# nvlong21/Lightweight-face-detection-CenterNet

Measured on AMD Instinct MI355X. Metric: images/sec at 640x640 batch inference, higher is better.
Workload: dtype bf16; 1 GPU; BASELINE configs[1]: batch=64 640x640 bf16 on 1 MI355X per rank, forward + top-100 peak decode; synthetic uint8 images resident in HBM, calibrated synthetic weights (seed 0); 2 context(s) per GPU, batch k on context k mod 2; batch_per_gpu=64, global_batch=64, topk=100, parallelism=dp1, contexts_per_gpu=2, input_buffers=4

## Files before the change

lightweight-face-detection-centernet_amd/csrc/cf_common.h:

```cpp
#pragma once
#include <hip/hip_runtime.h>
#include <stdint.h>
#include <stdlib.h>

typedef uint16_t bf16_t;

typedef __attribute__((ext_vector_type(4))) float f32x4;
typedef __attribute__((ext_vector_type(16))) float f32x16;
typedef __attribute__((ext_vector_type(8))) short bf16x8_t;
typedef __attribute__((ext_vector_type(4))) uint32_t u32x4;
typedef __attribute__((ext_vector_type(2))) uint32_t u32x2;

#define CF_WAVE 64

__device__ __forceinline__ float bf16_to_f32(uint32_t bits16) { return __uint_as_float(bits16 << 16); }
__device__ __forceinline__ float bf16lo(uint32_t packed) { return __uint_as_float(packed << 16); }
__device__ __forceinline__ float bf16hi(uint32_t packed) { return __uint_as_float(packed & 0xffff0000u); }

__device__ __forceinline__ uint32_t pack_bf16x2(float lo, float hi) {
    uint32_t r;
    asm("v_cvt_pk_bf16_f32 %0, %1, %2" : "=v"(r) : "v"(lo), "v"(hi));
    return r;
}

__device__ __forceinline__ float fast_rcp(float x) { return __builtin_amdgcn_rcpf(x); }

__device__ __forceinline__ float swish_f(float x) {
    return x * fast_rcp(1.0f + __expf(-x));
}
__device__ __forceinline__ float relu_f(float x) { return fmaxf(x, 0.0f); }

typedef __attribute__((ext_vector_type(2))) float f32x2;
__device__ __forceinline__ f32x2 swish2(f32x2 x) {
    const f32x2 t = x * -1.44269504088896341f;
    f32x2 e; e.x = __builtin_amdgcn_exp2f(t.x); e.y = __builtin_amdgcn_exp2f(t.y);
    const f32x2 den = e + 1.0f;
    f32x2 r; r.x = __builtin_amdgcn_rcpf(den.x); r.y = __builtin_amdgcn_rcpf(den.y);
    return x * r;
}
static constexpr float kCfNegLog2e = -1.44269504088896341f, kCfNegLn2 = -0.69314718055994531f;
template <bool PRE> __device__ __forceinline__ f32x2 swish2_sel(f32x2 x) {
    if constexpr (PRE) {
        f32x2 e; e.x = __builtin_amdgcn_exp2f(x.x); e.y = __builtin_amdgcn_exp2f(x.y);
        const f32x2 den = e + 1.0f;
        f32x2 r; r.x = __builtin_amdgcn_rcpf(den.x); r.y = __builtin_amdgcn_rcpf(den.y);
        return x * r;
    } else {
        return swish2(x);
    }
}
__device__ __forceinline__ f32x2 fma2(f32x2 a, f32x2 b, f32x2 c) { return __builtin_elementwise_fma(a, b, c); }
template <int ACT, int N> __device__ __forceinline__ void act_arr(float* v) {
    if constexpr (ACT == 1) {
#pragma unroll
        for (int e = 0; e < N; e += 2) {
            f32x2 x2; x2.x = v[e]; x2.y = v[e + 1];
            const f32x2 y2 = swish2(x2);
            v[e] = y2.x; v[e + 1] = y2.y;
        }
    } else if constexpr (ACT == 2) {
#pragma unroll
        for (int e = 0; e < N; ++e) v[e] = relu_f(v[e]);
    }
}
template <int ACT> __device__ __forceinline__ float act_f(float x) {
    if constexpr (ACT == 1) return swish_f(x);
    else if constexpr (ACT == 2) return relu_f(x);
    else return x;
}

template <typename T> struct Elem;
template <> struct Elem<float> {
    static constexpr int PER16 = 4;
};
template <> struct Elem<bf16_t> {
    static constexpr int PER16 = 8;
};

struct sp32_t { float v; };
template <> struct Elem<sp32_t> {
    static constexpr int PER16 = 4;
};

template <typename T> __device__ __forceinline__ void unpack16(const u32x4& c, float* f);
template <> __device__ __forceinline__ void unpack16<float>(const u32x4& c, float* f) {
    f[0] = __uint_as_float(c.x); f[1] = __uint_as_float(c.y);
// ... 92 lines not shown
typedef __attribute__((ext_vector_type(8))) uint32_t u32x8_t;
__device__ __forceinline__ void dot8_first(float* A, const u32x8_t& W, const u32x4& E0, const u32x4& E1) {
    asm("v_dot2_f32_f16 %0, %8, %16, 0\n\t"
        "v_dot2_f32_f16 %1, %9, %17, 0\n\t"
        "v_dot2_f32_f16 %2, %10, %18, 0\n\t"
        "v_dot2_f32_f16 %3, %11, %19, 0\n\t"
        "v_dot2_f32_f16 %4, %12, %20, 0\n\t"
        "v_dot2_f32_f16 %5, %13, %21, 0\n\t"
        "v_dot2_f32_f16 %6, %14, %22, 0\n\t"
        "v_dot2_f32_f16 %7, %15, %23, 0\n\t"
        "s_nop 2"
        : "=&v"(A[0]), "=&v"(A[1]), "=&v"(A[2]), "=&v"(A[3]), "=&v"(A[4]), "=&v"(A[5]), "=&v"(A[6]), "=&v"(A[7])
        : "s"(W[0]), "s"(W[1]), "s"(W[2]), "s"(W[3]), "s"(W[4]), "s"(W[5]), "s"(W[6]), "s"(W[7]),
          "v"(E0.x), "v"(E0.y), "v"(E0.z), "v"(E0.w), "v"(E1.x), "v"(E1.y), "v"(E1.z), "v"(E1.w));
}

__device__ __forceinline__ void cf_sync_lds_dma() {
    asm volatile("s_waitcnt vmcnt(0)" ::: "memory");
    __syncthreads();
}

template <int N> __device__ __forceinline__ void cf_sync_lds_dma_keep() {
    static_assert(N >= 0 && N <= 63, "vmcnt field");
    asm volatile("s_waitcnt vmcnt(%0)" :: "n"(N) : "memory");
    __syncthreads();
}

template <int DIV, int N, int SH = 16>
struct MulShiftDiv {
    static constexpr unsigned MUL = ((1u << SH) + DIV - 1) / DIV;
    static constexpr bool exact() {
        for (unsigned v = 0; v < (unsigned)N; ++v) if (((v * MUL) >> SH) != v / DIV) return false;
        return true;
    }
    static_assert((unsigned long long)N * MUL < (1ull << 32) && N < (1 << 24) && MUL < (1u << 24) && exact(), "24-bit multiply, exact quotient");
    static __device__ __forceinline__ unsigned div(unsigned v) { return (v * MUL) >> SH; }
};

typedef __amdgpu_buffer_rsrc_t cf_rsrc_t;
typedef __attribute__((ext_vector_type(4))) unsigned int cf_v4u;
constexpr unsigned CF_OOB = 0x80000000u;
__device__ __forceinline__ cf_rsrc_t cf_rsrc(const void* base, unsigned bytes) {
    return __builtin_amdgcn_make_buffer_rsrc(const_cast<void*>(base), 0, (int)bytes, 0x00020000);
}
__device__ __forceinline__ u32x4 cf_bload16(cf_rsrc_t r, unsigned off) {
    return __builtin_bit_cast(u32x4, __builtin_amdgcn_raw_buffer_load_b128(r, (int)off, 0, 0));
}
__device__ __forceinline__ uint32_t cf_bload4(cf_rsrc_t r, unsigned off) {
    return (uint32_t)__builtin_amdgcn_raw_buffer_load_b32(r, (int)off, 0, 0);
}
__device__ __forceinline__ void cf_bstore16(const u32x4& v, cf_rsrc_t r, unsigned off) {
    __builtin_amdgcn_raw_buffer_store_b128(__builtin_bit_cast(cf_v4u, v), r, (int)off, 0, 0);
}

template <int KS>
struct HaloDeal {
    static_assert(KS == 3 || KS == 5, "an even halo height");
    static constexpr int IH = 16 + KS - 1, IWQ = 5, NRP = IH / 2, NBLK = KS == 3 ? 3 : 4;
    static __device__ __forceinline__ int side_pairs(int w) { return w == 2 ? 4 : NRP - 4; }
    static __device__ __forceinline__ bool pixel(int w, int t, int pl, int& ty, int& tx) {
        const int tq = pl >> 3, hh = (pl >> 2) & 1, x = pl & 3;
        bool live = true;
        if (t < 2) {
            ty = 2 * (4 * t + w) + hh; tx = 4 * tq + x;
        } else if constexpr (KS == 3) {
            const bool side = w >= 2;
            const int lp = 2 * tq + (x >> 1);
            live = side ? lp < side_pairs(w) : tq < 2;
            ty = (side ? 2 * (4 * (w - 2) + lp) : 16) + hh;
            tx = side ? 16 + (x & 1) : 8 * w + 4 * tq + x;
        } else if (t == 2) {
            const bool side = w >= 2;
            ty = 2 * (side ? 4 * (w - 2) + tq : 8 + w) + hh;
            tx = side ? 16 + x : 4 * tq + x;
        } else {
            live = w >= 2 && tq == 0;
            ty = 2 * (6 + w) + hh; tx = 16 + x;
        }
        ty = live ? ty : 0; tx = live ? tx : 0;
        return live;
    }
};

template <int S, int TOH, int TOW, int IWP>
struct LaneMap {
    static constexpr int NPIX = TOH * TOW, PPX = S == 1 ? NPIX / 2 : NPIX, WPP = (PPX + 63) / 64, NSLOT = WPP * 64;
    static constexpr int ROWW = S == 1 ? TOW / 2 : TOW;
    static_assert(ROWW <= 64 && TOH <= 256, "entry packing: 6 bits of x, 9 bits of y below the idle flag");
    uint16_t v[NSLOT];
    static constexpr int pair_index(int r) {
        const int oy = r / ROWW, oxh = r - oy * ROWW;
        return S == 1 ? oy * (IWP / 2) + oxh : oy * IWP + oxh;
    }
    constexpr LaneMap() : v() {
        constexpr int NG = NSLOT / 16;
        int bucket[16][PPX] = {}; int cnt[16] = {}, used[16] = {};
        for (int r = 0; r < PPX; ++r) { const int b = pair_index(r) & 15; bucket[b][cnt[b]++] = r; }
        int slot[NSLOT] = {};
        for (int g = 0; g < NG; ++g)
            for (int b = 0; b < 16; ++b) slot[g * 16 + b] = used[b] < cnt[b] ? bucket[b][used[b]++] : -1;
        for (int b = 0; b < 16; ++b)
            while (used[b] < cnt[b]) {
                int s = 0; while (slot[s] >= 0) ++s;
                slot[s] = bucket[b][used[b]++];
            }
        for (int g = 0; g < NG; ++g)
            for (int j = 0; j < 16; ++j) {
                const int hw = g & 3;
                const int base = (hw & 1) ? (j < 8 ? 4 + j : j < 12 ? 16 + (j - 8) : 28 + (j - 12))
                                          : (j < 4 ? j : j < 8 ? 12 + (j - 4) : 20 + (j - 8));
                const int lane = base + (hw >> 1) * 32;
                const int r = slot[g * 16 + j];
                const int rc = r >= 0 ? r : cnt[j] > 0 ? bucket[j][0] : 0;
                const int oy = rc / ROWW, oxh = rc - oy * ROWW;
                v[(g >> 2) * 64 + lane] = (uint16_t)((r < 0 ? 0x8000 : 0) | (oy << 6) | oxh);
            }
    }
};

__device__ __forceinline__ int lds_group_pixel(int pl) {
    return pl < 4 ? pl : pl < 12 ? pl + 12 : pl < 16 ? pl - 8 : pl < 20 ? pl + 8 : pl < 28 ? pl - 12 : pl;
}

__device__ __forceinline__ void xcd_tile_order(unsigned& bx, unsigned& by, unsigned& bz) {
    const unsigned gx = gridDim.x, gy = gridDim.y, n = gx * gy * gridDim.z;
    unsigned l = blockIdx.x + gx * (blockIdx.y + gy * blockIdx.z);
    if ((n & 7u) == 0u) l = (l & 7u) * (n >> 3) + (l >> 3);
    bx = l % gx; l /= gx; by = l % gy; bz = l / gy;
}

static inline int cf_env_int(const char* name, int dflt) { const char* v = getenv(name); return v ? atoi(v) : dflt; }
#ifdef CF_EXPERIMENTS
static inline int cf_ab_int(const char* name, int dflt) { return cf_env_int(name, dflt); }
#else
static inline int cf_ab_int(const char*, int dflt) { return dflt; }
#endif

template <auto KFN, typename... A>
static inline hipError_t launch_lds(dim3 grid, dim3 blk, size_t lds, hipStream_t s, const A&... args) {
    if (lds > 64 * 1024) {
        static thread_local size_t raised_dev[32] = {};
        int dev = 0; (void)hipGetDevice(&dev);
        size_t& raised = raised_dev[dev & 31];
        if (raised < lds) {
            hipError_t e = hipFuncSetAttribute(reinterpret_cast<const void*>(KFN), hipFuncAttributeMaxDynamicSharedMemorySize, (int)lds);
            if (e != hipSuccess) return e;
            raised = lds;
        }
    }
    hipLaunchKernelGGL(KFN, grid, blk, lds, s, args...);
    return hipGetLastError();
}

template <typename E, size_t N, typename Match>
static inline const E* pick_variant(const E (&table)[N], int want, Match&& match) {
    const E* base = nullptr;
    for (const E& e : table)
        if (match(e)) {
            if (e.var == want) return &e;
            if (e.var == 0) base = &e;
        }
    return base;
}

static inline uint16_t host_f32_to_bf16(float f) {
    uint32_t u; __builtin_memcpy(&u, &f, 4);
// ... 41 lines not shown
```

lightweight-face-detection-centernet_amd/csrc/cf_mbconv2.hip:

```cpp
#include "cf_exp.h"
#include "cf_common.h"
#include "cf_kernels.h"
#include <cstdlib>
#include <type_traits>

namespace cf {

typedef __attribute__((ext_vector_type(8))) __bf16 mfma_bf16x8;
typedef __attribute__((ext_vector_type(8))) uint32_t u32x8;
typedef __attribute__((ext_vector_type(2))) __fp16 f16x2;
#define CF_AS4 __attribute__((address_space(4)))

static inline int slot_channel2(int nb, int i) {
    int h = (i >> 2) & 1;
    int r = (i & 3) + 4 * (i >> 3);
    return nb * 32 + h * 16 + r;
}

static inline uint16_t host_f32_to_f16(float f) {
    uint32_t u; __builtin_memcpy(&u, &f, 4);
    const uint32_t sign = (u >> 16) & 0x8000u;
    const int32_t exp = (int32_t)((u >> 23) & 0xff) - 127 + 15;
    uint32_t man = u & 0x7fffffu;
    if (((u >> 23) & 0xff) == 0xff) return (uint16_t)(sign | 0x7c00u | (man ? 0x200u : 0));
    if (exp >= 31) return (uint16_t)(sign | 0x7bffu);
    if (exp <= 0) {
        if (exp < -10) return (uint16_t)sign;
        man |= 0x800000u;
        const int shift = 14 - exp;
        uint32_t half = man >> shift;
        const uint32_t rem = man & ((1u << shift) - 1), mid = 1u << (shift - 1);
        if (rem > mid || (rem == mid && (half & 1))) ++half;
        return (uint16_t)(sign | half);
    }
    uint32_t half = ((uint32_t)exp << 10) | (man >> 13);
    const uint32_t rem = man & 0x1fffu;
    if (rem > 0x1000u || (rem == 0x1000u && (half & 1))) ++half;
    if (half >= 0x7c00u) half = 0x7bffu;
    return (uint16_t)(sign | half);
}

typedef __attribute__((ext_vector_type(2))) _Float16 hf2;
__device__ __forceinline__ void dot2c(float& acc, uint32_t w, uint32_t e) {
    acc = __builtin_amdgcn_fdot2(__builtin_bit_cast(hf2, w), __builtin_bit_cast(hf2, e), acc, false);
}

__device__ __forceinline__ f32x2 swish2_prescaled(f32x2 u) {
    f32x2 e; e.x = __builtin_amdgcn_exp2f(u.x); e.y = __builtin_amdgcn_exp2f(u.y);
    const f32x2 den = e + 1.0f;
    f32x2 r; r.x = __builtin_amdgcn_rcpf(den.x); r.y = __builtin_amdgcn_rcpf(den.y);
    return u * r;
}
static constexpr float kNegLog2e = -1.44269504088896341f, kNegLn2 = -0.69314718055994531f;

#define CF_DOT8_ACC(A, W, E0, E1)                                                                        \
    dot2c(A[0], W[0], E0.x); dot2c(A[1], W[1], E0.y); dot2c(A[2], W[2], E0.z); dot2c(A[3], W[3], E0.w);  \
    dot2c(A[4], W[4], E1.x); dot2c(A[5], W[5], E1.y); dot2c(A[6], W[6], E1.z); dot2c(A[7], W[7], E1.w)
#define CF_DOT8_Z(A, W, E0, E1)                                                                          \
    do { _Pragma("unroll") for (int i_ = 0; i_ < 8; ++i_) A[i_] = 0.0f; CF_DOT8_ACC(A, W, E0, E1); } while (0)
#define CF_DOT8(FIRST, A, W, E0, E1)                                                                     \
    do { if constexpr (FIRST) dot8_first(A, W, E0, E1); else { CF_DOT8_ACC(A, W, E0, E1); } } while (0)

#ifndef CF_WDIRECT_COND
#define CF_WDIRECT_COND (KS == 5 && S == 2 && NW == 3)
#endif
template <int KS, int S, int HC, int TOH, int TOW, int JX, int NW>
struct Px {
    static constexpr int IH = (TOH - 1) * S + KS, IW0 = (TOW - 1) * S + KS, IWP = (IW0 + 1) & ~1;
    static constexpr int IPX = IH * IWP, NIB = (IPX + 31) / 32, NPAIR = IPX / 2;
    static constexpr int NT = (KS + 1) / 2, NPARW = S == 1 ? 2 : 1;
    static constexpr int NPIX = TOH * TOW, PPX = S == 1 ? NPIX / 2 : NPIX, WPP = (PPX + 63) / 64;
    static constexpr int NPP = NPARW * WPP, KG = NW / NPP;
    static constexpr int NBE = (HC + 31) / 32, HALF = HC / 16, JS = HALF / KG;
    static constexpr bool PART = (HC % 32 == 16);
    static constexpr int NBF = HC / 32;
    static constexpr int PITCH = HC * 4 + 16;
    static constexpr int WXB = (NBF * JX + (PART ? 1 : 0)) * 1024;
    static_assert(!PART || JX <= 2, "half block needs Cin <= 32");
    static constexpr int EBYTES = NIB * 16 * PITCH;
    static constexpr int RED = (KG - 1) * NPP * 64 * 64;
    static constexpr bool WDIRECT = CF_WDIRECT_COND;
    static constexpr int WLDS = WDIRECT ? 0 : 2 * WXB;
    static constexpr int LDS = (EBYTES + WLDS) > RED ? (EBYTES + WLDS) : RED;
    static_assert(NPP * KG == NW && TOW % 2 == 0, "tile / wave geometry");
    static_assert(HC % 16 == 0 && JS * KG == HALF, "hidden chunk / k-group geometry");
};

#ifndef CF_XRELOAD_COND
#define CF_XRELOAD_COND (KS == 5 && S == 2 && NBO == 1 && NW == 3)
#endif
template <int KS, int S, int NBO, bool RESID, int NW, int JX, int HC, int TOH, int TOW, int MODE = 0>
__global__ __launch_bounds__(NW * 64) void mbconv_px_kernel(MbParams p) {
    typedef Px<KS, S, HC, TOH, TOW, JX, NW> G;
    constexpr bool FAST = MODE != 0, FAST_LD = (MODE & 1) != 0, FAST_WR = (MODE & 2) != 0;
    static_assert(!FAST || (!RESID && !G::PART), "MODE != 0: no residual, no 16-channel half block");
    constexpr int IWP = G::IWP, IPX = G::IPX, NIB = G::NIB, NPAIR = G::NPAIR, NT = G::NT, NPARW = G::NPARW;
    constexpr int NPP = G::NPP, KG = G::KG, NBF = G::NBF, HALF = G::HALF, JS = G::JS, PITCH = G::PITCH, WXB = G::WXB;
    constexpr bool PART = G::PART;
    extern __shared__ __attribute__((aligned(16))) char smem[];
    char* E = smem;
    char* Wst = smem + G::EBYTES;

    const int tid = threadIdx.x, lane = tid & 63;
    const int wave = __builtin_amdgcn_readfirstlane(tid >> 6);
    const int pl = lane & 31, h = lane >> 5;
    unsigned tbx = blockIdx.x, tby = blockIdx.y, tbz = blockIdx.z;
    if (p.nw) xcd_tile_order(tbx, tby, tbz);
    const int ox0 = tbx * TOW, oy0 = tby * TOH, b = tbz;
    const int nq = p.nq;
    const int pp = wave % NPP, jg = wave / NPP;

    const int par = S == 1 ? pp / G::WPP : 0;
    static constexpr LaneMap<S, TOH, TOW, IWP> kLanes{};
    const int lm0 = (S == 1 ? pp - par * G::WPP : pp) * 64;
    auto tile_pixel = [&](int blk, int lane31, int& oy, int& ox) -> bool {
        const uint32_t e = kLanes.v[lm0 + blk * 32 + lane31];
        oy = (e >> 6) & 0x1ff;
        ox = S == 1 ? 2 * (int)(e & 63) + par : (int)(e & 63);
        return (e & 0x8000u) == 0;
    };
    int dy, dx; tile_pixel(h, pl, dy, dx);
    const unsigned e_pix = (unsigned)(((dy * S) * IWP + (dx * S - par)) / 2) * (unsigned)PITCH;

    f32x16 acc[2][NBO];
#pragma unroll
    for (int k = 0; k < 2; ++k)
#pragma unroll
        for (int i = 0; i < NBO; ++i)
#pragma unroll
            for (int r = 0; r < 16; ++r) acc[k][i][r] = 0.0f;

    const char* xbase = (const char*)p.x + (size_t)b * p.Hin * p.Win * p.Cin * 2;
    const unsigned rowbytes = (unsigned)p.Cin * 2;

    auto stage_weights = [&](int q) {
        char* dst = Wst + (q & 1) * WXB;
        const char* srcx = (const char*)p.wexp + (size_t)q * WXB;
        for (int c = wave; c < WXB / 1024; c += NW)
            __builtin_amdgcn_global_load_lds((const __attribute__((address_space(1))) void*)(srcx + c * 1024 + lane * 16),
                                             (__attribute__((address_space(3))) void*)(dst + c * 1024), 16, 0, 0);
    };

    constexpr int MAXI = (NIB + NW - 1) / NW;
    constexpr bool XRELOAD = CF_XRELOAD_COND;
    u32x4 xf[MAXI][JX];
    u32x4 xh[PART ? MAXI : 1][2];
    typedef MulShiftDiv<IWP, MAXI * NW * 32> HD;
    const unsigned ip0 = (unsigned)(wave * 32 + pl);
    const int gy0 = oy0 * S - p.pad_lo, gx0 = ox0 * S - p.pad_lo;
    const unsigned hlim = (unsigned)min(p.Hin, gy0 + G::IH);
    const unsigned lbase = (((unsigned)b * (unsigned)p.Hin + (unsigned)gy0) * (unsigned)p.Win + (unsigned)gx0) * rowbytes + (unsigned)(h * JX * 16);
    const unsigned pitch24 = ((unsigned)p.Win * rowbytes) & 0xffffffu, rowb24 = rowbytes & 0xffffffu;
    const unsigned oobh = (h && (p.Cin & 8)) ? CF_OOB : 0u;
    const cf_rsrc_t xr = cf_rsrc(p.x, FAST_LD ? (unsigned)p.B * (unsigned)p.Hin * (unsigned)p.Win * rowbytes : 0u);
    auto load_x = [&]() {
    if constexpr (FAST_LD) {
#pragma unroll
        for (int t = 0; t < MAXI; ++t) {
            const unsigned ip = ip0 + (unsigned)(t * NW * 32);
            const unsigned iy = HD::div(ip), ix = ip - iy * (unsigned)IWP;
            const bool valid = (unsigned)(gy0 + (int)iy) < hlim && (unsigned)(gx0 + (int)ix) < (unsigned)p.Win;
            const unsigned off = valid ? iy * pitch24 + (ix * rowb24 + lbase) : CF_OOB;
#pragma unroll
            for (int j = 0; j < JX; ++j) xf[t][j] = cf_bload16(xr, (j == JX - 1 ? (off | oobh) : off) + j * 16);
        }
        return;
    }
#pragma unroll
    for (int t = 0; t < MAXI; ++t) {
        const int ib = wave + NW * t;
        const int ip = ib * 32 + pl;
        const int ipc = ip < IPX ? ip : IPX - 1;
        const int iy = ipc / IWP, ix = ipc - iy * IWP;
        const int gy = oy0 * S - p.pad_lo + iy, gx = ox0 * S - p.pad_lo + ix;
        const bool valid = ip < IPX && (unsigned)gy < (unsigned)p.Hin && (unsigned)gx < (unsigned)p.Win;
        const int cy = min(max(gy, 0), p.Hin - 1), cx = min(max(gx, 0), p.Win - 1);
        const unsigned off = ((unsigned)cy * (unsigned)p.Win + (unsigned)cx) * rowbytes + (unsigned)(h * JX * 16);
#pragma unroll
        for (int j = 0; j < JX; ++j) {
            const bool vj = valid && (h * JX + j) * 8 < p.Cin;
            const u32x4 v = ld16(xbase + off + j * 16);
            xf[t][j].x = vj ? v.x : 0u; xf[t][j].y = vj ? v.y : 0u;
            xf[t][j].z = vj ? v.z : 0u; xf[t][j].w = vj ? v.w : 0u;
        }
    }

    if constexpr (PART) {
#pragma unroll
        for (int t = 0; t < MAXI; ++t)
#pragma unroll
            for (int sub = 0; sub < 2; ++sub) {
                const int ib = wave + NW * t;
                const int ip = ib * 32 + sub * 16 + (lane & 15), kg = lane >> 4;
                const int ipc = ip < IPX ? ip : IPX - 1;
                const int iy = ipc / IWP, ix = ipc - iy * IWP;
                const int gy = oy0 * S - p.pad_lo + iy, gx = ox0 * S - p.pad_lo + ix;
                const bool valid = ip < IPX && (unsigned)gy < (unsigned)p.Hin && (unsigned)gx < (unsigned)p.Win && kg * 8 < p.Cin;
                const int cy = min(max(gy, 0), p.Hin - 1), cx = min(max(gx, 0), p.Win - 1);
                const u32x4 v = ld16(xbase + ((unsigned)cy * (unsigned)p.Win + (unsigned)cx) * rowbytes + (unsigned)(min(kg * 8, p.Cin - 8) * 2));
                xh[t][sub].x = valid ? v.x : 0u; xh[t][sub].y = valid ? v.y : 0u;
                xh[t][sub].z = valid ? v.z : 0u; xh[t][sub].w = valid ? v.w : 0u;
            }
    }
    };
    if constexpr (!XRELOAD) load_x();

    constexpr int VP = (IPX - 32 * (NIB - 1)) / 2;
    auto expand_block = [&](auto lastb, int ib, const u32x4* xfr, const u32x4* xhr, const char* wx) {
        constexpr bool LASTB = decltype(lastb)::value && VP < 16;
        if constexpr (PART) {
            const u32x4 wv = ld16(wx + (NBF * JX * 64 + lane) * 16);
            char* ecol = E + (NBF * 32 + (lane & 15)) * 4 + (unsigned)(ib * 16 + 2 * (lane >> 4)) * (unsigned)PITCH;
#pragma unroll
            for (int sub = 0; sub < 2; ++sub) {
                f32x4 a4 = {0.0f, 0.0f, 0.0f, 0.0f};
                a4 = __builtin_amdgcn_mfma_f32_16x16x32_bf16(__builtin_bit_cast(mfma_bf16x8, xhr[sub]),
                                                             __builtin_bit_cast(mfma_bf16x8, wv), a4, 0, 0, 0);
#pragma unroll
                for (int t = 0; t < 2; ++t) {
                    if (LASTB && sub * 8 + t >= VP) continue;
                    f32x2 x2; x2.x = a4[2 * t]; x2.y = a4[2 * t + 1];
                    const f32x2 y2 = swish2_prescaled(x2);
                    *reinterpret_cast<uint32_t*>(ecol + (sub * 8 + t) * PITCH) =
                        __builtin_bit_cast(uint32_t, __builtin_amdgcn_cvt_pkrtz(y2.x, y2.y));
                }
            }
        }
#pragma unroll
        for (int nbl = 0; nbl < NBF; ++nbl) {
            f32x16 a;
#pragma unroll
            for (int r = 0; r < 16; ++r) a[r] = 0.0f;
            const char* wb = wx + (nbl * JX * 64 + lane) * 16;
#pragma unroll
            for (int j = 0; j < JX; ++j) {
                const u32x4 wv = ld16(wb + j * 1024);
                a = __builtin_amdgcn_mfma_f32_32x32x16_bf16(__builtin_bit_cast(mfma_bf16x8, xfr[j]),
                                                            __builtin_bit_cast(mfma_bf16x8, wv), a, 0, 0, 0);
            }
            const int ch = nbl * 32 + pl;
            char* ecol = E + ch * 4 + (unsigned)(ib * 16 + 2 * h) * (unsigned)PITCH;
            uint32_t d[8];
#pragma unroll
            for (int t = 0; t < 8; ++t) {
                if (LASTB && (t & 1) + 4 * (t >> 1) >= VP) continue;
                f32x2 x2; x2.x = a[2 * t]; x2.y = a[2 * t + 1];
                const f32x2 y2 = swish2_prescaled(x2);
                d[t] = __builtin_bit_cast(uint32_t, __builtin_amdgcn_cvt_pkrtz(y2.x, y2.y));
            }
#pragma unroll
            for (int t = 0; t < 8; ++t) {
                if (LASTB && (t & 1) + 4 * (t >> 1) >= VP) continue;
                *reinterpret_cast<uint32_t*>(ecol + ((t & 1) + 4 * (t >> 1)) * PITCH) = d[t];
            }
        }
    };

    const CF_AS4 u32x8* wtab = (const CF_AS4 u32x8*)p.wdw;

    auto dw_chunk = [&](int q, int c) -> u32x4 {
        float a8[8];
        const CF_AS4 u32x8* wq = wtab + (p.nw < 0 ? (size_t)0 : (size_t)(((q * NPARW + par) * (HC / 8) + c) * KS) * NT);
        const char* eb = E + e_pix + c * 32;
        if constexpr (KS == 3) {
        u32x8 wa[KS * NT];
#pragma unroll
        for (int i = 0; i < KS * NT; ++i) wa[i] = wq[i];
        u32x4 en[NT][2];
#pragma unroll
        for (int t = 0; t < NT; ++t) { en[t][0] = ld16(eb + t * PITCH); en[t][1] = ld16(eb + t * PITCH + 16); }
#pragma unroll
        for (int ky = 0; ky < KS; ++ky) {
            u32x4 ec[NT][2];
#pragma unroll
            for (int t = 0; t < NT; ++t) { ec[t][0] = en[t][0]; ec[t][1] = en[t][1]; }
            if (ky + 1 < KS) {
#pragma unroll
                for (int t = 0; t < NT; ++t) {
                    const char* et = eb + ((ky + 1) * (IWP / 2) + t) * PITCH;
                    en[t][0] = ld16(et); en[t][1] = ld16(et + 16);
                }
            }
#pragma unroll
            for (int t = 0; t < NT; ++t) {
                const u32x8 wv = wa[ky * NT + t];
                if (ky == 0 && t == 0) { CF_DOT8(true, a8, wv, ec[t][0], ec[t][1]); }
                else { CF_DOT8(false, a8, wv, ec[t][0], ec[t][1]); }
            }
        }
        } else {
        u32x8 wn[NT]; u32x4 en[NT][2];
#pragma unroll
        for (int t = 0; t < NT; ++t) { wn[t] = wq[t]; en[t][0] = ld16(eb + t * PITCH); en[t][1] = ld16(eb + t * PITCH + 16); }
#pragma unroll
        for (int ky = 0; ky < KS; ++ky) {
            u32x8 wc[NT]; u32x4 ec[NT][2];
#pragma unroll
            for (int t = 0; t < NT; ++t) { wc[t] = wn[t]; ec[t][0] = en[t][0]; ec[t][1] = en[t][1]; }
            if (ky + 1 < KS) {
#pragma unroll
                for (int t = 0; t < NT; ++t) {
                    const char* et = eb + ((ky + 1) * (IWP / 2) + t) * PITCH;
                    wn[t] = wq[(ky + 1) * NT + t]; en[t][0] = ld16(et); en[t][1] = ld16(et + 16);
                }
            }
#pragma unroll
            for (int t = 0; t < NT; ++t) {
                if (ky == 0 && t == 0) { CF_DOT8_Z(a8, wc[t], ec[t][0], ec[t][1]); }
                else { CF_DOT8(false, a8, wc[t], ec[t][0], ec[t][1]); }
            }
        }
        }
#pragma unroll
        for (int i = 0; i < 8; i += 2) {
            f32x2 u; u.x = a8[i]; u.y = a8[i + 1];
            const f32x2 y = swish2_prescaled(u);
            a8[i] = y.x; a8[i + 1] = y.y;
        }
        return pack16<bf16_t>(a8);
    };

    if constexpr (!G::WDIRECT) stage_weights(0);
    for (int q = 0; q < nq; ++q) {
        const char* wx = G::WDIRECT ? (const char*)p.wexp + (size_t)q * WXB : Wst + (q & 1) * WXB;
        if constexpr (XRELOAD) load_x();
        cf_sync_lds_dma();

#pragma unroll
        for (int t = 0; t < MAXI; ++t) {
            const int ib = wave + NW * t;
            if (t == (NIB - 1) / NW && ib == NIB - 1) expand_block(std::true_type{}, ib, xf[t], xh[PART ? t : 0], wx);
            else if (ib < NIB) expand_block(std::false_type{}, ib, xf[t], xh[PART ? t : 0], wx);
        }
        __syncthreads();
        if (!G::WDIRECT && q + 1 < nq) stage_weights(q + 1);

#pragma unroll
        for (int j = 0; j < HALF; ++j) {
            if (KG > 1 && (j / JS) != jg) continue;
            u32x4 wpc[NBO];
#pragma unroll
            for (int i = 0; i < NBO; ++i)
                wpc[i] = ld16((const char*)p.wproj + ((((size_t)i * nq + q) * HALF + j) * 64 + lane) * 16);
            const u32x4 dA = dw_chunk(q, j), dB = dw_chunk(q, HALF + j);
            u32x4 x0, x1;
            {
                auto s0 = __builtin_amdgcn_permlane32_swap(dA.x, dB.x, false, false); x0.x = s0[0]; x1.x = s0[1];
                auto s1 = __builtin_amdgcn_permlane32_swap(dA.y, dB.y, false, false); x0.y = s1[0]; x1.y = s1[1];
                auto s2 = __builtin_amdgcn_permlane32_swap(dA.z, dB.z, false, false); x0.z = s2[0]; x1.z = s2[1];
                auto s3 = __builtin_amdgcn_permlane32_swap(dA.w, dB.w, false, false); x0.w = s3[0]; x1.w = s3[1];
            }
#pragma unroll
            for (int i = 0; i < NBO; ++i) {
                acc[0][i] = __builtin_amdgcn_mfma_f32_32x32x16_bf16(__builtin_bit_cast(mfma_bf16x8, wpc[i]),
                                                                    __builtin_bit_cast(mfma_bf16x8, x0), acc[0][i], 0, 0, 0);
                acc[1][i] = __builtin_amdgcn_mfma_f32_32x32x16_bf16(__builtin_bit_cast(mfma_bf16x8, wpc[i]),
                                                                    __builtin_bit_cast(mfma_bf16x8, x1), acc[1][i], 0, 0, 0);
            }
        }
    }

    if constexpr (KG > 1) {
        float* red = reinterpret_cast<float*>(smem) + (size_t)(pp * 64 + lane) * 16;
        constexpr int GSTRIDE = NPP * 64 * 16;
#pragma unroll
        for (int k = 0; k < 2; ++k)
#pragma unroll
            for (int i = 0; i < NBO; ++i) {
                __syncthreads();
                if (jg > 0) {
#pragma unroll
                    for (int g = 0; g < 4; ++g) {
                        float t[4];
#pragma unroll
                        for (int e = 0; e < 4; ++e) t[e] = acc[k][i][g * 4 + e];
                        st16(red + (jg - 1) * GSTRIDE + g * 4, pack16<float>(t));
                    }
                }
                __syncthreads();
                if (jg == 0) {
#pragma unroll
                    for (int gk = 0; gk < KG - 1; ++gk)
#pragma unroll
                        for (int g = 0; g < 4; ++g) {
                            float t[4];
                            unpack16<float>(ld16(red + gk * GSTRIDE + g * 4), t);
#pragma unroll
                            for (int e = 0; e < 4; ++e) acc[k][i][g * 4 + e] += t[e];
                        }
                }
            }
        if (jg > 0) return;
    }

    if constexpr (FAST_WR) {
        const cf_rsrc_t yr = cf_rsrc(p.y, (unsigned)p.B * (unsigned)p.Hout * (unsigned)p.Wout * (unsigned)p.Cout * 2u);
        const unsigned opix00 = ((unsigned)b * (unsigned)p.Hout + (unsigned)oy0) * (unsigned)p.Wout + (unsigned)ox0;
        const unsigned cob24 = ((unsigned)p.Cout * 2u) & 0xffffffu, opitch24 = ((unsigned)p.Wout * cob24) & 0xffffffu;
        const unsigned obase = opix00 * cob24 + (unsigned)(h * 32);
#pragma unroll
        for (int k = 0; k < 2; ++k) {
            int oy, ox;
            const bool livepx = tile_pixel(k, pl, oy, ox);
            const bool live = livepx && oy0 + oy < p.Hout && ox0 + ox < p.Wout;
            const unsigned off = (unsigned)oy * opitch24 + ((unsigned)ox * cob24 + obase);
#pragma unroll
            for (int i = 0; i < NBO; ++i)
#pragma unroll
                for (int g = 0; g < 2; ++g) {
                    float v[8];
#pragma unroll
                    for (int e = 0; e < 8; ++e) v[e] = acc[k][i][g * 8 + e];
                    const bool ok = live && i * 32 + h * 16 + g * 8 < p.Cout;
                    cf_bstore16(pack16<bf16_t>(v), yr, (ok ? off : CF_OOB) + (unsigned)(i * 64 + g * 16));
                }
        }
        return;
    }
#pragma unroll
    for (int k = 0; k < 2; ++k) {
        int oy, ox;
        const bool livepx = tile_pixel(k, pl, oy, ox);
        const int gy = oy0 + oy, gx = ox0 + ox;
        if (!livepx || gy >= p.Hout || gx >= p.Wout) continue;
        const size_t opix = ((size_t)b * p.Hout + gy) * p.Wout + gx;
#pragma unroll
        for (int i = 0; i < NBO; ++i) {
            const int cb = i * 32 + h * 16;
#pragma unroll
            for (int g = 0; g < 2; ++g) {
                const int ch = cb + g * 8;
                if (ch >= p.Cout) break;
                float v[8];
#pragma unroll
                for (int e = 0; e < 8; ++e) v[e] = acc[k][i][g * 8 + e];
                if constexpr (RESID) {
                    float r[8];
                    unpack16<bf16_t>(ld16((const char*)p.x + (opix * p.Cin + ch) * 2), r);
#pragma unroll
                    for (int e = 0; e < 8; ++e) v[e] = r[e] + v[e];
                }
                st16((char*)p.y + (p.yblock ? blk_off(opix, p.Cout / 8, ch / 8) : (opix * p.Cout + ch) * 2), pack16<bf16_t>(v));
            }
        }
    }
}


#ifndef CF_ILP_TU
template <int KS, int S, int HC, int TOH, int TOW, int JX>
struct Xd {
    static constexpr int IH = (TOH - 1) * S + KS, IW0 = (TOW - 1) * S + KS, IWP = (IW0 + 1) & ~1;
    static constexpr int IPX = IH * IWP, NIB = (IPX + 31) / 32;
    static constexpr int NT = (KS + 1) / 2, NPARW = S == 1 ? 2 : 1;
    static constexpr int NPIX = TOH * TOW, PPX = S == 1 ? NPIX / 2 : NPIX;
    static constexpr int WPP = (PPX + 63) / 64, NW = NPARW * WPP;
    static constexpr int NBE = HC / 32, PITCH = HC * 4 + 16, WXB = NBE * JX * 1024;
    static constexpr int EBYTES = NIB * 16 * PITCH, LDS = EBYTES + WXB;
    static_assert(HC % 32 == 0 && TOW % 2 == 0, "hidden chunk / tile geometry");
};

template <int KS, int S, int JX, int HC, int TOH, int TOW>
__global__ __launch_bounds__((Xd<KS, S, HC, TOH, TOW, JX>::NW) * 64) void expdw_px_kernel(MbParams p) {
    typedef Xd<KS, S, HC, TOH, TOW, JX> G;
    constexpr int IWP = G::IWP, IPX = G::IPX, NIB = G::NIB, NT = G::NT, NPARW = G::NPARW, NW = G::NW;
    constexpr int NBE = G::NBE, PITCH = G::PITCH, WXB = G::WXB, PPX = G::PPX, WPP = G::WPP;
    extern __shared__ __attribute__((aligned(16))) char smem[];
    char* E = smem;
    char* Wst = smem + G::EBYTES;

    const int tid = threadIdx.x, lane = tid & 63;
    const int wave = __builtin_amdgcn_readfirstlane(tid >> 6);
    const int pl = lane & 31, h = lane >> 5;
    const int tiles_x = (p.Wout + TOW - 1) / TOW;
    const int tyi = blockIdx.x / tiles_x, txi = blockIdx.x - tyi * tiles_x;
    const int ox0 = txi * TOW, oy0 = tyi * TOH, b = blockIdx.z;
    const int grp = blockIdx.y;

    {
        const char* srcx = (const char*)p.wexp + (size_t)grp * WXB;
        for (int c = wave; c < WXB / 1024; c += NW)
            __builtin_amdgcn_global_load_lds((const __attribute__((address_space(1))) void*)(srcx + c * 1024 + lane * 16),
                                             (__attribute__((address_space(3))) void*)(Wst + c * 1024), 16, 0, 0);
    }
    const char* xbase = (const char*)p.x + (size_t)b * p.Hin * p.Win * p.Cin * 2;
    const unsigned rowbytes = (unsigned)p.Cin * 2;
    auto load_x = [&](int ib, u32x4* xf) -> bool {
        const int ip = ib * 32 + pl;
        const int ipc = ip < IPX ? ip : IPX - 1;
        const int iy = ipc / IWP, ix = ipc - iy * IWP;
        const int gy = oy0 * S - p.pad_lo + iy, gx = ox0 * S - p.pad_lo + ix;
        const int cy = min(max(gy, 0), p.Hin - 1), cx = min(max(gx, 0), p.Win - 1);
        if (p.xblock) {
            const char* xb = (const char*)p.x + blk_off(((size_t)b * p.Hin + cy) * p.Win + cx, p.Cin / 8, h * JX);
#pragma unroll
            for (int j = 0; j < JX; ++j) xf[j] = ld16(xb + j * 512);
        } else {
            const unsigned off = ((unsigned)cy * (unsigned)p.Win + (unsigned)cx) * rowbytes + (unsigned)(h * JX * 16);
#pragma unroll
            for (int j = 0; j < JX; ++j) xf[j] = ld16(xbase + off + j * 16);
        }
        return ip < IPX && (unsigned)gy < (unsigned)p.Hin && (unsigned)gx < (unsigned)p.Win;
    };
    const bool last_in = (h * JX + JX - 1) * 8 < p.Cin;
    auto mask_x = [&](u32x4* xf, bool valid) {
#pragma unroll
        for (int j = 0; j < JX; ++j) {
            const bool vj = j == JX - 1 ? (valid && last_in) : valid;
            xf[j].x = vj ? xf[j].x : 0u; xf[j].y = vj ? xf[j].y : 0u; xf[j].z = vj ? xf[j].z : 0u; xf[j].w = vj ? xf[j].w : 0u;
        }
    };
    u32x4 xa[JX];
    bool va = false;
    if (wave < NIB) va = load_x(wave, xa);
    cf_sync_lds_dma();
    mask_x(xa, va);

    for (int ib = wave; ib < NIB; ib += NW) {
        u32x4 xn[JX];
        const bool more = ib + NW < NIB;
        bool vn = false;
        if (more) vn = load_x(ib + NW, xn);
#pragma unroll
        for (int nbl = 0; nbl < NBE; ++nbl) {
            f32x16 a;
// ... 59 lines not shown
            }
#pragma unroll
            for (int t = 0; t < NT; ++t) {
                if (ky == 0 && t == 0) { CF_DOT8_Z(a8, wc[t], ec[t][0], ec[t][1]); }
                else { CF_DOT8(false, a8, wc[t], ec[t][0], ec[t][1]); }
            }
        }
#pragma unroll
        for (int i = 0; i < 8; i += 2) {
            f32x2 u; u.x = a8[i]; u.y = a8[i + 1];
            const f32x2 y = swish2_prescaled(u) * kNegLn2;
            a8[i] = y.x; a8[i + 1] = y.y;
        }
        if (store) st16(out + c * ostep, pack16<bf16_t>(a8));
    }
}

struct XdEntry {
    int k, s, jx, hc, toh, tow, var, lds_bytes, nt, nparw, nw;
    hipError_t (*fn)(hipStream_t, const MbParams&);
};
template <int KS, int S, int JX, int HC, int TOH, int TOW>
static hipError_t xd_launch_t(hipStream_t s, const MbParams& p) {
    typedef Xd<KS, S, HC, TOH, TOW, JX> G;
    dim3 grid(((p.Wout + TOW - 1) / TOW) * ((p.Hout + TOH - 1) / TOH), p.hid / HC, p.B), blk(G::NW * 64);
    set_kernel_tag("void cf::expdw_px_kernel<%d, %d, %d, %d, %d, %d>(cf::MbParams)", KS, S, JX, HC, TOH, TOW);
    return launch_lds<expdw_px_kernel<KS, S, JX, HC, TOH, TOW>>(grid, blk, G::LDS, s, p);
}
#define XD(V, KS, S, JX, HC, TOH, TOW)                                                                             \
    {KS, S, JX, HC, TOH, TOW, V, Xd<KS, S, HC, TOH, TOW, JX>::LDS, Xd<KS, S, HC, TOH, TOW, JX>::NT, Xd<KS, S, HC, TOH, TOW, JX>::NPARW, \
     Xd<KS, S, HC, TOH, TOW, JX>::NW, &xd_launch_t<KS, S, JX, HC, TOH, TOW>}
static const XdEntry kXdTable[] = {
    XD(0, 5, 2, 6, 32, 10, 20),
    XD(0, 5, 1, 10, 32, 10, 20),
    XD(0, 3, 1, 10, 32, 10, 20),
    XD(0, 5, 1, 4, 32, 10, 40),
    XD(0, 5, 1, 6, 32, 10, 40),
#include CF_EXP_INC(cf_mbconv2_0)
};
#undef XD
static const XdEntry* xd_find(int k, int s, int jx) {
    static const int want = cf_ab_int("CF_XD_VARIANT", 0);
    return pick_variant(kXdTable, want, [&](const XdEntry& e) { return e.k == k && e.s == s && e.jx == jx; });
}

MbGeom expdw_geometry(int dtype, int Cin, int hid, int k, int s) {
    if (dtype != 1) return expdw_f32_geometry(dtype, Cin, hid, k, s);
    MbGeom g = expdw_mx_geometry(dtype, Cin, hid, k, s);
    if (g.ok) return g;
    static const bool off = cf_ab_int("CF_XD_KIND", 1) == 0;
    if (off || dtype != 1 || (Cin % 8) || hid == Cin) return g;
    const int jx = (Cin * 2 / 16 + 1) / 2;
    const XdEntry* e = xd_find(k, s, jx);
    if (!e || hid % e->hc) return g;
    g.ok = true; g.kind = XD_PX; g.S = s;
    g.JX = jx; g.NBO = 0; g.HC = e->hc; g.nq = hid / e->hc; g.NBE = e->hc / 32; g.HALF = 0;
    g.rowb = e->hc * 4 + 16;
    g.lds_bytes = (size_t)e->lds_bytes;
    g.wexp_bytes = (size_t)g.nq * g.NBE * g.JX * 64 * 16;
    g.wdw_floats = (size_t)g.nq * e->nparw * (g.HC / 8) * k * e->nt * 8;
    g.wproj_bytes = 0;
    return g;
}
hipError_t expdw_launch(hipStream_t s, int, const MbParams& p) {
    const XdEntry* e = xd_find(p.k, p.s, p.JX);
    if (!e || e->hc != p.HC) return hipErrorInvalidValue;
    return e->fn(s, p);
}

struct Mb2Entry {
    int k, s, jx, hc, nbo, res, toh, tow, nw, var;
    int lds_bytes, nt, nparw, nbe, half, wxb;
    hipError_t (*fn)(hipStream_t, const MbParams&);
};

#endif
template <int KS, int S, int NBO, bool RESID, int NW, int JX, int HC, int TOH, int TOW>
hipError_t mb2_launch_t(hipStream_t s, const MbParams& p) {
    constexpr int LDS = Px<KS, S, HC, TOH, TOW, JX, NW>::LDS;
    dim3 grid((p.Wout + TOW - 1) / TOW, (p.Hout + TOH - 1) / TOH, p.B), blk(NW * 64);
    static const bool xcd_on = cf_ab_int("CF_MB2_XCD", 0) == 1;
    MbParams q = p; q.nw = xcd_on ? 1 : 0;
    set_kernel_tag("void cf::mbconv_px_kernel<%d, %d, %d, %s, %d, %d, %d, %d, %d>(cf::MbParams)", KS, S, NBO, RESID ? "true" : "false", NW, JX, HC, TOH, TOW);
    if constexpr (KS == 3 && S == 2 && NBO == 1 && !RESID && JX == 1 && HC == 32 && TOH == 8 && TOW == 16 && NW == 4) {
        static const bool fast_on = cf_ab_int("CF_FRONT_MODE", 1) != 0;
        const size_t mx = (size_t)p.B * p.Hin * p.Win, my = (size_t)p.B * p.Hout * p.Wout;
        const bool small = mx * p.Cin * 2 < ((size_t)1 << 31) && my * p.Cout * 2 < ((size_t)1 << 31) && (size_t)p.Win * p.Cin * 2 < ((size_t)1 << 24) &&
                           (size_t)p.Wout * p.Cout * 2 < ((size_t)1 << 24);
        if (fast_on && small && !p.yblock) return launch_lds<mbconv_px_kernel<KS, S, NBO, RESID, NW, JX, HC, TOH, TOW, 3>>(grid, blk, LDS, s, q);
    }
    return launch_lds<mbconv_px_kernel<KS, S, NBO, RESID, NW, JX, HC, TOH, TOW>>(grid, blk, LDS, s, q);
}

#define CF_MB2_ILP_INSTANCES(X) \
    X(3, 2, 1, false, 4, 1, 32, 8, 16)   \
    X(3, 2, 2, false, 4, 2, 32, 8, 16)
#ifdef CF_ILP_TU
#define CF_X(KS, S, NBO, RES, NW, JX, HC, TOH, TOW) template hipError_t mb2_launch_t<KS, S, NBO, RES, NW, JX, HC, TOH, TOW>(hipStream_t, const MbParams&);
CF_MB2_ILP_INSTANCES(CF_X)
#undef CF_X
#else
#define CF_X(KS, S, NBO, RES, NW, JX, HC, TOH, TOW) extern template hipError_t mb2_launch_t<KS, S, NBO, RES, NW, JX, HC, TOH, TOW>(hipStream_t, const MbParams&);
CF_MB2_ILP_INSTANCES(CF_X)
#undef CF_X
#endif

#ifndef CF_ILP_TU
#define MB2(V, KS, S, JX, HC, NBO, RES, TOH, TOW, NW)                                                               \
    {KS, S, JX, HC, NBO, RES, TOH, TOW, NW, V, Px<KS, S, HC, TOH, TOW, JX, NW>::LDS, Px<KS, S, HC, TOH, TOW, JX, NW>::NT, \
     Px<KS, S, HC, TOH, TOW, JX, NW>::NPARW, Px<KS, S, HC, TOH, TOW, JX, NW>::NBE, Px<KS, S, HC, TOH, TOW, JX, NW>::HALF,  \
     Px<KS, S, HC, TOH, TOW, JX, NW>::WXB, &mb2_launch_t<KS, S, NBO, (RES != 0), NW, JX, HC, TOH, TOW>}
static const Mb2Entry kMb2Table[] = {
    MB2(0, 3, 2, 1, 32, 1, 0, 8, 16, 4),
    MB2(0, 3, 1, 2, 48, 1, 1, 16, 16, 4),
    MB2(0, 5, 2, 2, 48, 1, 0, 8, 8, 3),
    MB2(0, 5, 1, 2, 64, 1, 1, 8, 16, 4),
    MB2(0, 3, 2, 2, 32, 2, 0, 8, 16, 4),
    MB2(0, 3, 1, 4, 64, 2, 1, 8, 16, 4),
    MB2(0, 5, 1, 4, 64, 3, 0, 8, 16, 4),
    MB2(0, 5, 1, 6, 64, 3, 1, 8, 16, 4),
#include CF_EXP_INC(cf_mbconv2_1)
};
#undef MB2

static const Mb2Entry* mb2_find(int k, int s, int jx, int nbo, int res) {
    static const int want = cf_ab_int("CF_MB2_VARIANT", 0);
    return pick_variant(kMb2Table, want, [&](const Mb2Entry& e) { return e.k == k && e.s == s && e.jx == jx && e.nbo == nbo && e.res == res; });
}

bool mb2_geometry(MbGeom& g, int Cin, int hid, int Cout, int k, int s) {
    static const bool off = cf_ab_int("CF_MB_KIND", 1) == 0;
    if (off) return false;
    const int jx = (Cin * 2 / 16 + 1) / 2, nbo = (Cout + 31) / 32;
    const Mb2Entry* e = mb2_find(k, s, jx, nbo, (Cin == Cout && s == 1) ? 1 : 0);
    if (!e || hid % e->hc) return false;
    g.ok = true; g.kind = MB_PX; g.S = s;
    g.JX = jx; g.NBO = nbo; g.HC = e->hc; g.nq = hid / e->hc; g.NBE = e->nbe; g.HALF = e->half;
    g.rowb = e->hc * 4 + 16;
    g.lds_bytes = (size_t)e->lds_bytes;
    g.wexp_bytes = (size_t)g.nq * e->wxb;
    g.wdw_floats = (size_t)g.nq * e->nparw * (g.HC / 8) * k * e->nt * 8;
    g.wproj_bytes = (size_t)g.NBO * g.nq * g.HALF * 64 * 16;
    return true;
}

void mb2_pack_weights(int, const MbGeom& g, int Cin, int hid, int Cout, int k, const float* we, const float* wd, const float* wp,
                      void* wexp_host, float* wdw_host, void* wproj_host) {
    const int NCx = Cin * 2 / 16, NT = (k + 1) / 2, NPARW = g.S == 1 ? 2 : 1;
    __builtin_memset(wexp_host, 0, g.wexp_bytes);
    if (wproj_host) __builtin_memset(wproj_host, 0, g.wproj_bytes);
    uint32_t* wt = reinterpret_cast<uint32_t*>(wdw_host);
    for (int q = 0; q < g.nq; ++q) {
        const bool part = g.kind == MB_PX && (g.HC % 32 == 16);
        const int nbf = part ? g.HC / 32 : g.NBE;
        const size_t wxb = ((size_t)nbf * g.JX + (part ? 1 : 0)) * 1024;
        for (int nbl = 0; nbl < nbf; ++nbl)
            for (int j = 0; j < g.JX; ++j)
                for (int lane = 0; lane < 64; ++lane) {
                    const int n = lane & 31, hh = lane >> 5;
                    const int cl = nbl * 32 + n, c = hh * g.JX + j;
                    if (cl >= g.HC || c >= NCx) continue;
                    uint16_t* dst = (uint16_t*)((char*)wexp_host + (size_t)q * wxb + (((size_t)nbl * g.JX + j) * 64 + lane) * 16);
                    for (int e = 0; e < 8; ++e) dst[e] = host_f32_to_bf16(kNegLog2e * we[(size_t)(q * g.HC + cl) * Cin + (size_t)c * 8 + e]);
                }
        if (part)
            for (int lane = 0; lane < 64; ++lane) {
                const int n = lane & 15, kg = lane >> 4;
// ... 37 lines not shown
```

Before: 56470 images/s.

## Add half-tile edge path to mbconv kernel to skip dead columns

Adds an EDGE template variant of the fused mbconv kernel. When a tile's right half lies past the output width, it loads, expands and stores only the live half using a compact HalfDeal pixel mapping, and for stride 2 idles the dead wave's projection. It is enabled by default for the stride-1 residual layer (L31), with a compile-time yblock choice. The L30 layer is also routed into the existing fast-mode launch path. This trims wasted expand and MFMA work on edge tiles, at the cost of more template instantiations and divergent code on those tiles.

Result: no change. 56760 images/s (median of 5 runs) (+0.5%).

```diff
diff --git a/lightweight-face-detection-centernet_amd/csrc/cf_common.h b/lightweight-face-detection-centernet_amd/csrc/cf_common.h
--- a/lightweight-face-detection-centernet_amd/csrc/cf_common.h
+++ b/lightweight-face-detection-centernet_amd/csrc/cf_common.h
@@ -2,6 +2,7 @@
 #include <hip/hip_runtime.h>
 #include <stdint.h>
 #include <stdlib.h>
+#include <type_traits>
 
 typedef uint16_t bf16_t;
 
@@ -260,6 +261,28 @@
     }
 };
 
+template <int N, int I = 0, typename F>
+__device__ __forceinline__ void cf_static_for(F&& f) {
+    if constexpr (I < N) { f(std::integral_constant<int, I>{}); cf_static_for<N, I + 1>(f); }
+}
+
+template <int KS, int S, int TOH, int TOW, int NW>
+struct HalfDeal {
+    static constexpr int IH = (TOH - 1) * S + KS, IWP = ((TOW - 1) * S + KS + 1) & ~1, W2 = IWP / 2;
+    static constexpr int COLS = (TOW / 2 - 1) * S + KS, LPW = (COLS + 1) / 2, RH = (IH + 1) / 2;
+    static constexpr int NK = RH * LPW, NLB = (NK + 7) / 8, MAXT = (NLB + NW - 1) / NW, VP = NK - 8 * (NLB - 1);
+    static constexpr unsigned UPPER = (unsigned)(RH * W2);
+    typedef MulShiftDiv<LPW, MAXT * NW * 8> RowDiv;
+    static_assert(LPW < W2 && (2 * RH - 1) * W2 + LPW <= ((IH * IWP + 31) / 32) * 16, "row 2 RH - 1 stays inside the tile");
+    static __device__ __forceinline__ bool pixel(int lb, int pl, int& iy, int& ix) {
+        const unsigned t = ((unsigned)(pl >> 1) & 1u) + 2u * (unsigned)(pl >> 3), up = (unsigned)(pl >> 2) & 1u;
+        const unsigned k = (unsigned)lb * 8u + t, r = RowDiv::div(k);
+        iy = (int)(r + up * RH); ix = (int)(2 * (k - r * LPW) + (pl & 1));
+        return r < (unsigned)RH && iy < IH;
+    }
+    static __device__ __forceinline__ unsigned cell(unsigned k) { return k + (k / LPW) * (unsigned)(W2 - LPW); }
+};
+
 template <int S, int TOH, int TOW, int IWP>
 struct LaneMap {
     static constexpr int NPIX = TOH * TOW, PPX = S == 1 ? NPIX / 2 : NPIX, WPP = (PPX + 63) / 64, NSLOT = WPP * 64;
diff --git a/lightweight-face-detection-centernet_amd/csrc/cf_mbconv2.hip b/lightweight-face-detection-centernet_amd/csrc/cf_mbconv2.hip
--- a/lightweight-face-detection-centernet_amd/csrc/cf_mbconv2.hip
+++ b/lightweight-face-detection-centernet_amd/csrc/cf_mbconv2.hip
@@ -10,6 +10,11 @@
 typedef __attribute__((ext_vector_type(8))) uint32_t u32x8;
 typedef __attribute__((ext_vector_type(2))) __fp16 f16x2;
 #define CF_AS4 __attribute__((address_space(4)))
+#ifdef CF_EXPERIMENTS
+#define CF_EXPERIMENTS_ON true
+#else
+#define CF_EXPERIMENTS_ON false
+#endif
 
 static inline int slot_channel2(int nb, int i) {
     int h = (i >> 2) & 1;
@@ -89,11 +94,16 @@
 #ifndef CF_XRELOAD_COND
 #define CF_XRELOAD_COND (KS == 5 && S == 2 && NBO == 1 && NW == 3)
 #endif
-template <int KS, int S, int NBO, bool RESID, int NW, int JX, int HC, int TOH, int TOW, int MODE = 0>
+template <int KS, int S, int NBO, bool RESID, int NW, int JX, int HC, int TOH, int TOW, int MODE = 0, int EDGE = 0>
 __global__ __launch_bounds__(NW * 64) void mbconv_px_kernel(MbParams p) {
     typedef Px<KS, S, HC, TOH, TOW, JX, NW> G;
     constexpr bool FAST = MODE != 0, FAST_LD = (MODE & 1) != 0, FAST_WR = (MODE & 2) != 0;
     static_assert(!FAST || (!RESID && !G::PART), "MODE != 0: no residual, no 16-channel half block");
+    constexpr bool EDGE_ON = EDGE != 0, EDGE_DW = EDGE_ON && S == 2;
+    typedef HalfDeal<EDGE_ON ? KS : 3, EDGE_ON ? S : 1, EDGE_ON ? TOH : 8, EDGE_ON ? TOW : 16, EDGE_ON ? NW : 4> HT;
+    static_assert(HT::MAXT <= (G::NIB + NW - 1) / NW, "the half tile's X fragments fit the whole tile's registers");
+    static_assert(!EDGE_ON || (!FAST && !G::PART && !(CF_XRELOAD_COND)), "EDGE: the general addressing, whole 32-channel blocks, X in registers");
+    static_assert(!EDGE_DW || (G::WPP == 2 && TOH * TOW == 128), "EDGE, stride 2: the live half of the tile is one wave's 64 pixels");
     constexpr int IWP = G::IWP, IPX = G::IPX, NIB = G::NIB, NPAIR = G::NPAIR, NT = G::NT, NPARW = G::NPARW;
     constexpr int NPP = G::NPP, KG = G::KG, NBF = G::NBF, HALF = G::HALF, JS = G::JS, PITCH = G::PITCH, WXB = G::WXB;
     constexpr bool PART = G::PART;
@@ -113,8 +123,16 @@
     const int par = S == 1 ? pp / G::WPP : 0;
     static constexpr LaneMap<S, TOH, TOW, IWP> kLanes{};
     const int lm0 = (S == 1 ? pp - par * G::WPP : pp) * 64;
+    auto half_tile = [&]() -> bool {
+        int xe = ox0 + TOW / 2;
+        asm volatile("" : "+s"(xe));
+        return EDGE_ON && xe == p.Wout;
+    };
+    auto dw_idle = [&]() -> bool { return EDGE_DW && pp != 0 && half_tile(); };
+    static constexpr LaneMap<S, TOH, EDGE_DW ? TOW / 2 : TOW, IWP> kLanesH{};
     auto tile_pixel = [&](int blk, int lane31, int& oy, int& ox) -> bool {
-        const uint32_t e = kLanes.v[lm0 + blk * 32 + lane31];
+        uint32_t e = kLanes.v[lm0 + blk * 32 + lane31];
+        if constexpr (EDGE_DW) { if (half_tile()) e = pp != 0 ? 0x8000u : kLanesH.v[blk * 32 + lane31]; }
         oy = (e >> 6) & 0x1ff;
         ox = S == 1 ? 2 * (int)(e & 63) + par : (int)(e & 63);
         return (e & 0x8000u) == 0;
@@ -166,6 +184,27 @@
         }
         return;
     }
+    if constexpr (EDGE_ON) {
+        if (half_tile()) {
+            cf_static_for<HT::MAXT>([&](auto tc) {
+                constexpr int t = decltype(tc)::value;
+                int iy, ix;
+                const bool inside = HT::pixel(wave + NW * t, pl, iy, ix);
+                const int gy = oy0 * S - p.pad_lo + iy, gx = ox0 * S - p.pad_lo + ix;
+                const bool valid = inside && (unsigned)gy < (unsigned)p.Hin && (unsigned)gx < (unsigned)p.Win;
+                const int cy = min(max(gy, 0), p.Hin - 1), cx = min(max(gx, 0), p.Win - 1);
+                const unsigned off = ((unsigned)cy * (unsigned)p.Win + (unsigned)cx) * rowbytes + (unsigned)(h * JX * 16);
+#pragma unroll
+                for (int j = 0; j < JX; ++j) {
+                    const bool vj = valid && (h * JX + j) * 8 < p.Cin;
+                    const u32x4 v = ld16(xbase + off + j * 16);
+                    xf[t][j].x = vj ? v.x : 0u; xf[t][j].y = vj ? v.y : 0u;
+                    xf[t][j].z = vj ? v.z : 0u; xf[t][j].w = vj ? v.w : 0u;
+                }
+            });
+            return;
+        }
+    }
 #pragma unroll
     for (int t = 0; t < MAXI; ++t) {
         const int ib = wave + NW * t;
@@ -206,8 +245,11 @@
     if constexpr (!XRELOAD) load_x();
 
     constexpr int VP = (IPX - 32 * (NIB - 1)) / 2;
-    auto expand_block = [&](auto lastb, int ib, const u32x4* xfr, const u32x4* xhr, const char* wx) {
-        constexpr bool LASTB = decltype(lastb)::value && VP < 16;
+    int zq = 0;
+    auto expand_block = [&](auto lastb, auto halft, int ib, const u32x4* xfr, const u32x4* xhr, const char* wx) {
+        constexpr bool HALFT = decltype(halft)::value;
+        constexpr int VPB = HALFT ? HT::VP : VP;
+        constexpr bool LASTB = decltype(lastb)::value && VPB < (HALFT ? 8 : 16);
         if constexpr (PART) {
             const u32x4 wv = ld16(wx + (NBF * JX * 64 + lane) * 16);
             char* ecol = E + (NBF * 32 + (lane & 15)) * 4 + (unsigned)(ib * 16 + 2 * (lane >> 4)) * (unsigned)PITCH;
@@ -240,17 +282,25 @@
             }
             const int ch = nbl * 32 + pl;
             char* ecol = E + ch * 4 + (unsigned)(ib * 16 + 2 * h) * (unsigned)PITCH;
+            if constexpr (HALFT) {
+                const unsigned ln = __builtin_amdgcn_mbcnt_hi(~0u, __builtin_amdgcn_mbcnt_lo(~0u, (unsigned)zq));
+                ecol = E + (nbl * 32 + (ln & 31u)) * 4 + (ln >> 5) * (HT::UPPER * (unsigned)PITCH);
+            }
             uint32_t d[8];
 #pragma unroll
             for (int t = 0; t < 8; ++t) {
-                if (LASTB && (t & 1) + 4 * (t >> 1) >= VP) continue;
+                if (LASTB && (HALFT ? t : (t & 1) + 4 * (t >> 1)) >= VPB) continue;
                 f32x2 x2; x2.x = a[2 * t]; x2.y = a[2 * t + 1];
                 const f32x2 y2 = swish2_prescaled(x2);
                 d[t] = __builtin_bit_cast(uint32_t, __builtin_amdgcn_cvt_pkrtz(y2.x, y2.y));
             }
 #pragma unroll
             for (int t = 0; t < 8; ++t) {
-                if (LASTB && (t & 1) + 4 * (t >> 1) >= VP) continue;
+                if (LASTB && (HALFT ? t : (t & 1) + 4 * (t >> 1)) >= VPB) continue;
+                if constexpr (HALFT) {
+                    const unsigned c0 = __builtin_amdgcn_readfirstlane(HT::cell((unsigned)(ib * 8 + t)) * (unsigned)PITCH);
+                    *reinterpret_cast<uint32_t*>(ecol + c0) = d[t];
+                } else
                 *reinterpret_cast<uint32_t*>(ecol + ((t & 1) + 4 * (t >> 1)) * PITCH) = d[t];
             }
         }
@@ -326,11 +376,23 @@
         if constexpr (XRELOAD) load_x();
         cf_sync_lds_dma();
 
+        if (EDGE_ON && half_tile()) {
+            if constexpr (EDGE_ON) {
+                zq = p.nw < 0 ? q : 0;
+                cf_static_for<HT::MAXT>([&](auto tc) {
+                    constexpr int t = decltype(tc)::value;
+                    const int lb = wave + NW * t + zq;
+                    if (t == (HT::NLB - 1) / NW && lb == HT::NLB - 1) expand_block(std::true_type{}, std::true_type{}, lb, xf[t], xh[0], wx);
+                    else if (lb < HT::NLB) expand_block(std::false_type{}, std::true_type{}, lb, xf[t], xh[0], wx);
+                });
+            }
+        } else {
 #pragma unroll
         for (int t = 0; t < MAXI; ++t) {
             const int ib = wave + NW * t;
-            if (t == (NIB - 1) / NW && ib == NIB - 1) expand_block(std::true_type{}, ib, xf[t], xh[PART ? t : 0], wx);
-            else if (ib < NIB) expand_block(std::false_type{}, ib, xf[t], xh[PART ? t : 0], wx);
+            if (t == (NIB - 1) / NW && ib == NIB - 1) expand_block(std::true_type{}, std::false_type{}, ib, xf[t], xh[PART ? t : 0], wx);
+            else if (ib < NIB) expand_block(std::false_type{}, std::false_type{}, ib, xf[t], xh[PART ? t : 0], wx);
+        }
         }
         __syncthreads();
         if (!G::WDIRECT && q + 1 < nq) stage_weights(q + 1);
@@ -338,6 +400,7 @@
 #pragma unroll
         for (int j = 0; j < HALF; ++j) {
             if (KG > 1 && (j / JS) != jg) continue;
+            if (EDGE_DW && dw_idle()) continue;
             u32x4 wpc[NBO];
 #pragma unroll
             for (int i = 0; i < NBO; ++i)
@@ -417,6 +480,7 @@
         }
         return;
     }
+    const bool yblock = EDGE_ON ? EDGE == 2 : p.yblock != 0;
 #pragma unroll
     for (int k = 0; k < 2; ++k) {
         int oy, ox;
@@ -440,7 +504,7 @@
 #pragma unroll
                     for (int e = 0; e < 8; ++e) v[e] = r[e] + v[e];
                 }
-                st16((char*)p.y + (p.yblock ? blk_off(opix, p.Cout / 8, ch / 8) : (opix * p.Cout + ch) * 2), pack16<bf16_t>(v));
+                st16((char*)p.y + (yblock ? blk_off(opix, p.Cout / 8, ch / 8) : (opix * p.Cout + ch) * 2), pack16<bf16_t>(v));
             }
         }
     }
@@ -666,7 +730,23 @@
     static const bool xcd_on = cf_ab_int("CF_MB2_XCD", 0) == 1;
     MbParams q = p; q.nw = xcd_on ? 1 : 0;
     set_kernel_tag("void cf::mbconv_px_kernel<%d, %d, %d, %s, %d, %d, %d, %d, %d>(cf::MbParams)", KS, S, NBO, RESID ? "true" : "false", NW, JX, HC, TOH, TOW);
-    if constexpr (KS == 3 && S == 2 && NBO == 1 && !RESID && JX == 1 && HC == 32 && TOH == 8 && TOW == 16 && NW == 4) {
+    constexpr bool L30 = KS == 3 && S == 2 && NBO == 2 && !RESID && NW == 4 && JX == 2 && HC == 32 && TOH == 8 && TOW == 16;
+    constexpr bool L31 = KS == 3 && S == 1 && NBO == 2 && RESID && NW == 4 && JX == 4 && HC == 64 && TOH == 8 && TOW == 16;
+    if constexpr (L30 || L31) {
+#ifdef CF_EXPERIMENTS
+        static const int edge = cf_ab_int("CF_EDGE_MODE", 2);
+        const bool edge_on = (edge & (L30 ? 1 : 2)) != 0;
+#else
+        constexpr bool edge_on = L31;
+#endif
+        if constexpr (L31 || CF_EXPERIMENTS_ON) {
+            if (edge_on) {
+                if (p.yblock) return launch_lds<mbconv_px_kernel<KS, S, NBO, RESID, NW, JX, HC, TOH, TOW, 0, 2>>(grid, blk, LDS, s, q);
+                return launch_lds<mbconv_px_kernel<KS, S, NBO, RESID, NW, JX, HC, TOH, TOW, 0, 1>>(grid, blk, LDS, s, q);
+            }
+        }
+    }
+    if constexpr (L30 || (KS == 3 && S == 2 && NBO == 1 && !RESID && JX == 1 && HC == 32 && TOH == 8 && TOW == 16 && NW == 4)) {
         static const bool fast_on = cf_ab_int("CF_FRONT_MODE", 1) != 0;
         const size_t mx = (size_t)p.B * p.Hin * p.Win, my = (size_t)p.B * p.Hout * p.Wout;
         const bool small = mx * p.Cin * 2 < ((size_t)1 << 31) && my * p.Cout * 2 < ((size_t)1 << 31) && (size_t)p.Win * p.Cin * 2 < ((size_t)1 << 24) &&
```
